# SKA-INAF/caesar-yolo

Measured on AMD Instinct MI355X. Metric: 512x512 tiles/sec over 16k x 16k FITS, higher is better.
Workload: dtype f16

## Files before the change

caesar_yolo_amd/csrc/cy_extra.hip:

```cpp
#include "cy_kernels.h"
#include "cy_conv_dev.h"
#include <cstdlib>

namespace cy {

template <typename T> struct Vec8;
template <> struct Vec8<f16> { typedef f16 type __attribute__((ext_vector_type(8))); };
template <> struct Vec8<float> { typedef float type __attribute__((ext_vector_type(8))); };

template <bool SPLIT, typename T> __device__ __forceinline__ float ld1(const T* p, int lo) {
    if constexpr (SPLIT) return (float)p[0] + (float)p[lo]; else return (float)p[0];
}
template <bool SPLIT, typename T> __device__ __forceinline__ void st1(T* p, int lo, float v) {
    if constexpr (SPLIT) { const T h = (T)v; p[0] = h; p[lo] = (T)(v - (float)h); } else p[0] = (T)v;
}

constexpr int DW_PX = 4;
template <typename T, bool SPLIT = false>
__global__ __launch_bounds__(256) void dwconv3x3_kernel(const DwArgs a) {
    typedef typename Vec8<T>::type v8;
    const int cg = a.C / 8, xb = (a.W + DW_PX - 1) / DW_PX;
    const long total = (long)a.B * a.H * xb * cg;
    const long wg = a.xcd ? xcd_contiguous(blockIdx.x, gridDim.x) : blockIdx.x;
    for (long idx = wg * 256 + threadIdx.x; idx < total; idx += (long)gridDim.x * 256) {
// ... 225 lines not shown
        const int c = (int)(idx % cv) * V;
        const long pix = idx / cv;
        const int w = (int)(pix % a.W), h = (int)((pix / a.W) % a.H), b = (int)(pix / ((long)a.W * a.H));
        const T* base = reinterpret_cast<const T*>(a.src) + a.src_coff + c;
        vec m = *reinterpret_cast<const vec*>(base + (((long)b * a.H + h) * a.W + w) * a.ct);
#pragma unroll
        for (int dh = -2; dh <= 2; ++dh) {
            int hh = h + dh;
            hh = hh < 0 ? 0 : (hh >= a.H ? a.H - 1 : hh);
#pragma unroll
            for (int dw = -2; dw <= 2; ++dw) {
                if (dh == 0 && dw == 0) continue;
                int ww = w + dw;
                ww = ww < 0 ? 0 : (ww >= a.W ? a.W - 1 : ww);
                const vec v = *reinterpret_cast<const vec*>(base + (((long)b * a.H + hh) * a.W + ww) * a.ct);
#pragma unroll
                for (int j = 0; j < V; ++j) m[j] = v[j] > m[j] ? v[j] : m[j];
            }
        }
        *reinterpret_cast<vec*>(reinterpret_cast<T*>(a.dst) + pix * a.ct + a.dst_coff + c) = m;
    }
}

__global__ __launch_bounds__(256) void pool5_x3_kernel(const PoolArgs a) {
    const int cv = a.C / 8;
    const long total = (long)a.B * a.H * a.W * cv;
    for (long idx = (long)xcd_contiguous(blockIdx.x, gridDim.x) * 256 + threadIdx.x; idx < total; idx += (long)gridDim.x * 256) {
        const int c = (int)(idx % cv) * 8;
        const long pix = idx / cv;
        const int w = (int)(pix % a.W), h = (int)((pix / a.W) % a.H), b = (int)(pix / ((long)a.W * a.H));
        float m[8]; f16x8 mh, ml;
        bool first = true;
        for (int dh = -2; dh <= 2; ++dh)
            for (int dw = -2; dw <= 2; ++dw) {
                const int hh = h + dh, ww = w + dw;
                if ((unsigned)hh >= (unsigned)a.H || (unsigned)ww >= (unsigned)a.W) continue;
                const f16* sp = reinterpret_cast<const f16*>(a.src) + (((long)b * a.H + hh) * a.W + ww) * a.ct + a.src_coff + c;
                const f16x8 vh = *reinterpret_cast<const f16x8*>(sp), vl = *reinterpret_cast<const f16x8*>(sp + a.lo);
#pragma unroll
                for (int j = 0; j < 8; ++j) {
                    const float v = (float)vh[j] + (float)vl[j];
                    if (first || v > m[j]) { m[j] = v; mh[j] = vh[j]; ml[j] = vl[j]; }
                }
                first = false;
            }
        f16* dp = reinterpret_cast<f16*>(a.dst) + pix * a.ct + a.dst_coff + c;
// ... 43 lines not shown
```

caesar_yolo_amd/csrc/cy_kernels.h:

```cpp
#pragma once
#include <hip/hip_runtime.h>
#include <stdint.h>
#include <stdlib.h>
#include "cy_measure_jobs.h"
#include "cy_conv_plan.h"

namespace cy {

#ifndef CY_DEV_KNOBS
#define CY_DEV_KNOBS 0
#endif
inline int env_knob(const char* name, int dflt) { const char* e = getenv(name); return e ? atoi(e) : dflt; }
inline int dev_knob(const char* name, int dflt) { return CY_DEV_KNOBS ? env_knob(name, dflt) : dflt; }

template <auto Kernel> void lds_cap(size_t cap) {
    static bool done = false;
    if (done) return;
    (void)hipFuncSetAttribute(reinterpret_cast<const void*>(Kernel), hipFuncAttributeMaxDynamicSharedMemorySize, (int)cap);
    done = true;
}
template <auto Kernel, typename... A> hipError_t launch_lds(dim3 grid, dim3 block, size_t lds, size_t cap, hipStream_t s, A... args) {
    lds_cap<Kernel>(cap);
    hipLaunchKernelGGL(Kernel, grid, block, lds, s, args...);
    return hipGetLastError();
// ... 40 lines not shown
    int xcd;
};
struct AttnArgs {
    const void* qkv; int ct, coff; void* out; int out_ct, out_coff; int B, N, heads, kd, hd; float scale;
    int lo, out_lo;
};
hipError_t launch_dwconv(Precision p, const DwArgs& a, hipStream_t s);
hipError_t launch_attention(Precision p, const AttnArgs& a, hipStream_t s);

hipError_t launch_conv(Precision p, const ConvChoice& choice, const ConvArgs& a, hipStream_t s);
hipError_t launch_head_pair(Precision p, const ConvArgs& a, const ConvArgs& b, hipStream_t s);
void debug_read_stamps(unsigned long long* out8, bool reset);
void debug_read_wg_life(unsigned long long* out, int n);
void debug_read_wg_stamps(unsigned long long* out, int n);
void debug_read_pre_stamps(unsigned long long* out8, bool reset);
void debug_fastdiv(const double* d_a, const double* d_b, double* d_fast, double* d_ref, int n);
void debug_reduce(const double* d_val, const float* d_key, int nrows, int len, unsigned long long* d_out);
hipError_t launch_lds_fill(unsigned pattern, hipStream_t s, int* bytes);
hipError_t launch_stem(Precision p, const StemArgs& a, hipStream_t s);
hipError_t launch_stem_down(const StemDownArgs& a, hipStream_t s);
long stem_down_blocks(const StemDownArgs& a);
void pack_stem_weights2(const float* W, int cout, void* dst);
hipError_t launch_pool5(Precision p, const PoolArgs& a, hipStream_t s);

size_t packed_weight_bytes(Precision p, int cout, int cin, int k, int chunk_bytes = 128);
void pack_weights(Precision p, const float* W, int cout, int cin, int k, void* dst, int chunk_bytes = 128);
void pack_weights_fused2(const float* W2, int cout2, int cin2, void* dst);
int x3_passes(const float* W, int cout, int cin, int k, const float* scale);
size_t packed_weight_bytes_x3(int cout, int cin, int k, int chunk_bytes = 128, int passes = 3);
void pack_weights_x3(const float* W, int cout, int cin, int k, void* dst, float* oscale, int chunk_bytes = 128, int passes = 3, const float* scale = nullptr);
hipError_t launch_x3_split(const float* in, void* out, long npix, int C, hipStream_t s);
hipError_t launch_x3_merge(const void* in, float* out, long npix, int C, hipStream_t s);
void pack_stem_weights(const float* W, int cout, void* dst);
__device__ __forceinline__ int xcd_contiguous(int bid, int nwg) {
    const int q = nwg >> 3, r = nwg & 7, x = bid & 7;
    return (x < r ? x * (q + 1) : r * (q + 1) + (x - r) * q) + (bid >> 3);
}

struct DecodeArgs {
    const float* pred;
    int B, A, nc;
    int lvl_h[3], lvl_w[3];
    float conf;
    float* cand;
    int* cand_anchor;
    int* cand_count;
// ... 237 lines not shown
```

caesar_yolo_amd/csrc/cy_plan.cpp:

```cpp
#include "cy_plan.h"
#include <algorithm>
#include <cmath>
#include <map>

namespace cy {

namespace {
struct Scale { double d, w; int mc; };
bool scale_of(char s, Scale* o) {
    switch (s) {
        case 'n': *o = {0.33, 0.25, 1024}; return true;
        case 's': *o = {0.33, 0.50, 1024}; return true;
        case 'm': *o = {0.67, 0.75, 768}; return true;
        case 'l': *o = {1.00, 1.00, 512}; return true;
        case 'x': *o = {1.00, 1.25, 512}; return true;
    }
    return false;
}
int make_div8(double x) { return (int)std::ceil(x / 8.0) * 8; }

struct Builder {
    Plan p;
    std::map<std::string, int> idx;
    int T(int level, int C) { p.tensors.push_back({level, C}); return (int)p.tensors.size() - 1; }
// ... 337 lines not shown
    if (d2.k != 1 || d2.s != 1 || d2.cin != 256 || d2.cout > 256 || d2.cout % 16) return false;
    if (o.in1 >= 0 || o.up0 || o.res >= 0 || n.res >= 0 || n.c0 != 256) return false;
    if (p.tensors[o.out].level != p.tensors[n.out].level || n.out == o.out) return false;
    return readers_of(p, o.out) == 1;
}

bool box_branch(const Plan& p, size_t i) {
    if (i + 2 >= p.ops.size()) return false;
    const Op& o = p.ops[i]; const Op& n = p.ops[i + 1]; const Op& h = p.ops[i + 2];
    if (o.kind != OPK_CONV || !plain_conv_pair(o, n) || h.kind != OPK_CONV || h.conv < 0) return false;
    const ConvDesc& d0 = p.convs[o.conv]; const ConvDesc& d1 = p.convs[n.conv]; const ConvDesc& d2 = p.convs[h.conv];
    auto c3 = [](const ConvDesc& d) { return d.k == 3 && d.s == 1 && d.act && d.groups == 1 && d.cout == 64; };
    if (!c3(d0) || !c3(d1) || d1.cin != 64 || d0.cin % 64 || o.c0 != d0.cin || n.c0 != 64) return false;
    if (d2.k != 1 || d2.s != 1 || d2.act || d2.groups != 1 || d2.cin != 64 || d2.cout != 64) return false;
    if (o.in1 >= 0 || o.up0 || o.res >= 0 || n.res >= 0 || o.out_coff != 0 || n.out_coff != 0) return false;
    if (h.out >= 0 || h.pred_coff != 0 || h.in0 != n.out || h.in0_coff != 0 || h.c0 != 64 || h.in1 >= 0 || h.up0 || h.res >= 0) return false;
    if (p.tensors[o.out].C != 64 || p.tensors[n.out].C != 64 || o.out == n.out || o.in0 == o.out || o.in0 == n.out) return false;
    const int lev = p.tensors[o.in0].level;
    if (lev != 3 + h.pred_level || p.tensors[o.out].level != lev || p.tensors[n.out].level != lev) return false;
    int writers0 = 0, writers1 = 0;
    for (const Op& q : p.ops) { writers0 += q.out == o.out; writers1 += q.out == n.out; }
    return writers0 == 1 && writers1 == 1 && readers_of(p, o.out) == 1 && readers_of(p, n.out) == 1;
}
}

void mark_fusions(Plan& p) {
    for (size_t i = 0; i < p.ops.size(); ++i) {
        Op& o = p.ops[i];
        o.fuse = FUSE_NONE;
        if (o.box == 0 && box_branch(p, i)) { o.box = 1; p.ops[i + 1].box = 2; p.ops[i + 2].box = 3; }
        if (i + 1 >= p.ops.size()) continue;
        if (bneck_pair(p, i)) o.fuse = FUSE_BNECK_PAIR;
        else if (stem_down_pair(p, i)) o.fuse = FUSE_STEM_DOWN;
        else if (pw_pair(p, i)) o.fuse = FUSE_PW_PAIR;
    }
}

}
```

caesar_yolo_amd/csrc/cy_plan.h:

```cpp
#pragma once
#include <algorithm>
#include <cstddef>
#include <cstdint>
#include <cstring>
#include <string>
#include <vector>

namespace cy {

struct ConvDesc { std::string name; int cin, cout, k, s, act; int groups = 1; };

struct Tensor { int level; int C; };

enum OpKind { OPK_STEM = 0, OPK_CONV = 1, OPK_POOL = 2, OPK_DWCONV = 3, OPK_ATTN = 4 };

enum FuseMark { FUSE_NONE = 0, FUSE_STEM_DOWN, FUSE_PW_PAIR, FUSE_BNECK_PAIR };

struct Op {
    OpKind kind;
    int conv;
    int in0, in0_coff, c0, up0;
    int in1, in1_coff, c1;
    int out, out_coff;
    int res, res_coff;
    int pred_level, pred_coff;
    int p0 = 0, p1 = 0, p2 = 0, p3 = 0;
    FuseMark fuse = FUSE_NONE;
    int box = 0;
};

struct Plan {
    char scale; int nc;
    std::string arch = "yolov8";
    std::vector<ConvDesc> convs;
    std::vector<Tensor> tensors;
    std::vector<Op> ops;
    int feat_level[3];
    bool ok; std::string err;
};

Plan build_plan(char scale, int nc);
int py_round(double x);

struct Reader {
    const unsigned char* p; size_t n, o = 0; bool bad = false;
    uint32_t u32() { if (n - o < 4) { bad = true; return 0; } uint32_t v; memcpy(&v, p + o, 4); o += 4; return v; }
    std::string str(uint32_t len) { if (n - o < len) { bad = true; return ""; } std::string s((const char*)p + o, len); o += std::min<size_t>((len + (size_t)3) / 4 * 4, n - o); return s; }
    const float* f32(size_t cnt) { if ((n - o) / 4 < cnt) { bad = true; return nullptr; } const float* r = (const float*)(p + o); o += 4 * cnt; return r; }
};
struct FileHeader { bool v2 = false, has_flags = false, unsupported = false; uint32_t nconv = 0; std::vector<std::string> names; };
struct ConvRecord { ConvDesc d; const float* W; const float* b; const float* wscale; };
// ... 8 lines not shown
```

caesar_yolo_amd/csrc/cy_runtime.hip:

```cpp
#include "../../include/caesar_yolo_hip.h"
#include "cy_kernels.h"
#include "cy_measure_plan.h"
#include "cy_plan.h"
#include <algorithm>
#include <cmath>
#include <cstdio>
#include <cstdlib>
#include <cstring>
#include <string>
#include <vector>

using namespace cy;

struct DevConv { void* w = nullptr; float* bias = nullptr; size_t wbytes = 0; float* stem_w = nullptr; void* w32 = nullptr; size_t w32bytes = 0;
                 float* oscale = nullptr;
                 void* w2f = nullptr; size_t w2fbytes = 0;
                 int passes = 3;
                 float* dw_w = nullptr;
                 void* bneck = nullptr; };

enum MeasureStep { STEP_SOURCES = 0, STEP_ISLANDS, STEP_DEBLEND, STEP_FIT, STEP_BLEND, STEP_BACKGROUND, STEP_RENDER, STEP_RESIDUAL, STEP_PEAKS, STEP_ATROUS, STEP_APERTURE, STEP_PEAKFIT, STEP_COUNT };

struct DevOwner {
    std::vector<void*> p;
// ... 681 lines not shown
            }
            if (o.out < 0 && o.pred_coff == 0 && c->prec != PREC_F32 && knobs.head_pair && ch.variant == CONV_HEAD_1X1) {
                HeadPend& h = pend[o.pred_level];
                if (h.on) { cur_conv = h.conv; HIPCHK(c, launch_conv(c->prec, h.ch, h.a, s)); prof_done(h.ch.variant, h.flops); cur_conv = o.conv; }
                h.a = a; h.ch = ch; h.flops = flops; h.conv = o.conv; h.on = true;
                return CY_OK;
            }
            if (o.out < 0 && o.pred_coff == 64 && pend[o.pred_level].on) {
                HeadPend& h = pend[o.pred_level];
                h.on = false;
                if (head_pair_ok(c->prec, h.a, h.ch, a, ch, knobs)) {
                    HIPCHK(c, launch_head_pair(c->prec, h.a, a, s));
                    prof_done(CONV_HEAD_1X1, flops + h.flops);
                    return CY_OK;
                }
                cur_conv = h.conv; HIPCHK(c, launch_conv(c->prec, h.ch, h.a, s)); prof_done(h.ch.variant, h.flops); cur_conv = o.conv;
            }
            HIPCHK(c, launch_conv(c->prec, ch, a, s));
            prof_done(ch.variant, flops);
        }
        return CY_OK;
    };
    const size_t n_run = stop > 0 && (size_t)stop < p.ops.size() ? (size_t)stop : p.ops.size();
    size_t i = 0;
    for (; i < n_run; ++i) {
        bool fused = false;
        rc = run_op(p.ops[i], i + 1 < p.ops.size() ? &p.ops[i + 1] : nullptr, &fused);
        if (rc) return rc;
        if (fused) c->fused_last[i++] = 1;
    }
    c->ops_done = (int)(i < p.ops.size() ? i : p.ops.size());
    if (n_run < p.ops.size()) return CY_OK;
    for (HeadPend& h : pend)
        if (h.on) { h.on = false; cur_conv = h.conv; HIPCHK(c, launch_conv(c->prec, h.ch, h.a, s)); prof_done(h.ch.variant, h.flops); }
    if (box_sparse[0] || box_sparse[1] || box_sparse[2]) {
        HIPCHK(c, hipMemsetAsync(bx.L[0].map, 0xFF, (size_t)B * A * sizeof(int), s));
        HIPCHK(c, hipMemsetAsync(bx.L[0].counts, 0, 8 * sizeof(int), s));
        HIPCHK(c, launch_box_mark(bx, s));
        HIPCHK(c, launch_box_sparse(bx, s));
    }
    return CY_OK;
}

int cy_profile_enable(cy_ctx* c, int on) {
    if (!c) return CY_ERR_ARG;
    c->profiling = on != 0;
    c->prof_stride = on > 1 ? on : 1;
    c->fwd_calls = 0;
// ... 317 lines not shown
    if (!ch8(ct) || !ch8(src_coff) || !ch8(dst_coff) || src_coff + C > ct || dst_coff + C > ct)
        return fail(c, CY_ERR_ARG, "channel slice outside its tensor, or an offset / stride not a multiple of 8");
    if (d_src == d_dst && src_coff < dst_coff + C && dst_coff < src_coff + C) return fail(c, CY_ERR_ARG, "overlapping source and destination slices");
    HIPCHK(c, hipSetDevice(c->device));
    hipStream_t st = (hipStream_t)stream;
    const bool x3 = c->prec == PREC_F16X3;
    const int cm = x3 ? 2 : 1;
    const long npix = (long)B * H * W;
    DevOwner sc;
    void *src = const_cast<void*>(d_src), *dst = d_dst;
    hipError_t e = hipSuccess;
    if (x3) e = sc.split(d_dst, npix, ct, &dst, st);
    if (e == hipSuccess && x3) { if (d_src == d_dst) src = dst; else e = sc.split(d_src, npix, ct, &src, st); }
    if (e == hipSuccess) {
        PoolArgs a{};
        a.src = src; a.dst = dst; a.ct = cm * ct; a.src_coff = src_coff; a.dst_coff = dst_coff; a.lo = x3 ? ct : 0;
        a.C = C; a.B = B; a.H = H; a.W = W;
        e = launch_pool5(c->prec, a, st);
    }
    if (e == hipSuccess && x3) e = launch_x3_merge(dst, reinterpret_cast<float*>(d_dst), npix, ct, st);
    return entry_done(c, e, st);
}

int cy_debug_stamps(unsigned long long* out8, int reset) {
    if (!out8) return CY_ERR_ARG;
    if (reset <= -(1 << 20)) { debug_read_wg_life(out8, -reset - (1 << 20)); return CY_OK; }
    if (reset < 0) { debug_read_wg_stamps(out8, -reset); return CY_OK; }
    if (reset >= 2) debug_read_pre_stamps(out8, reset == 3);
    else debug_read_stamps(out8, reset != 0);
    return CY_OK;
}

int cy_debug_fastdiv(const double* d_a, const double* d_b, double* d_fast, double* d_ref, int n) {
    if (!d_a || !d_b || !d_fast || !d_ref || n < 1) return CY_ERR_ARG;
    debug_fastdiv(d_a, d_b, d_fast, d_ref, n);
    return hipGetLastError() == hipSuccess ? CY_OK : CY_ERR_HIP;
}

int cy_debug_reduce(const double* d_val, const float* d_key, int nrows, int len, unsigned long long* d_out) {
    if (!d_out || nrows < 1 || len < 0 || (len > 0 && (!d_val || !d_key))) return CY_ERR_ARG;
    debug_reduce(d_val, d_key, nrows, len, d_out);
    return hipGetLastError() == hipSuccess ? CY_OK : CY_ERR_HIP;
}

int cy_debug_lds_fill(cy_ctx* c, unsigned pattern32, void* stream) {
    if (!c) return CY_ERR_ARG;
// ... 741 lines not shown
```

caesar_yolo_amd/csrc/cy_sparse_box.hip:

```cpp
#include "cy_conv_dev.h"

namespace cy {

namespace {
constexpr int MI = 4, PG = 16 * MI;

__device__ __forceinline__ f16x8 to_mfma_order(const u32x4& v, int src4) {
    u32x4 r;
#pragma unroll
    for (int j = 0; j < 4; ++j) r[j] = (unsigned)__builtin_amdgcn_ds_bpermute(src4, (int)v[j]);
    return __builtin_bit_cast(f16x8, r);
}

template <bool WALK32, int TAPS>
__device__ __forceinline__ void walk(f32x4 (&acc)[4][MI], const unsigned (&xoff)[MI][TAPS], __amdgpu_buffer_rsrc_t rsx, __amdgpu_buffer_rsrc_t rsw,
                                     int nblocks, int lane) {
    static_assert(!WALK32 || TAPS == 9, "the 32-channel walk is the wide 3x3 kernel's");
    constexpr int NS = 2 * TAPS, RING = 3, CPAD = 128;
    const int lr = lane >> 2, lc = lane & 3;
    const int src4 = 4 * (4 * (lane & 15) + (lane >> 4));
    const unsigned wlane = WALK32 ? (unsigned)(lr * 64 + lc * 16) : (unsigned)(lr * 128 + lc * 16);
    u32x4 x[RING][MI], w[RING][4];
    auto load = [&](int slot, int cb, int u) {
        unsigned xs, ws;
// ... 75 lines not shown
        unsigned xoff[MI][9];
#pragma unroll
        for (int mi = 0; mi < MI; ++mi) {
            const int e = g * PG + mi * 16 + lr;
            const int p = e < n ? L.plist[e] : 0;
            const int b = p / HW, r = p - b * HW, y = r / L.W, x = r - y * L.W;
#pragma unroll
            for (int tap = 0; tap < 9; ++tap) {
                const int yy = y + tap / 3 - 1, xx = x + tap % 3 - 1;
                const bool ok = e < n && (unsigned)yy < (unsigned)L.H && (unsigned)xx < (unsigned)L.W;
                xoff[mi][tap] = ok ? (unsigned)((b * HW + yy * L.W + xx) * L.feat_ct + L.feat_coff + lc * 8) * 2u : CY_OOB;
            }
        }
        f32x4 acc[4][MI];
        zero(acc);
        walk<WALK32, 9>(acc, xoff, rsx, rsw, L.cin / 64, lane);
#pragma unroll
        for (int mi = 0; mi < MI; ++mi) {
            const int e = g * PG + mi * 16 + fr;
            if (e < n) act_store<PACKED>(acc, mi, bv, reinterpret_cast<f16*>(L.s1) + (size_t)e * 64 + fq * 16);
        }
    }
}
}

__global__ __launch_bounds__(256) void box_stage1_kernel(const BoxArgs a) {
    const BoxLevel& L = a.L[blockIdx.y];
    if (!L.sparse) return;
    const int lane = threadIdx.x & 63, wid = blockIdx.x * 4 + (threadIdx.x >> 6), nwaves = gridDim.x * 4;
    if (L.walk1 == BOX_WALK_WIDE) stage1<true, true>(L, wid, nwaves, lane);
    else if (L.walk1 == BOX_WALK_PP) stage1<false, false>(L, wid, nwaves, lane);
    else stage1<false, true>(L, wid, nwaves, lane);
}

__global__ __launch_bounds__(256) void box_stage2_kernel(const BoxArgs a) {
    const BoxLevel& L = a.L[blockIdx.y];
    if (!L.sparse) return;
    const int lane = threadIdx.x & 63, fr = lane & 15, fq = lane >> 4, wid = blockIdx.x * 4 + (threadIdx.x >> 6), nwaves = gridDim.x * 4;
    const int n = min(L.counts[1], L.cap), HW = L.H * L.W;
    const auto rsx = __builtin_amdgcn_make_buffer_rsrc(L.s1, 0, (unsigned)L.cap * 128u, 0x00020000);
    const auto rsw = __builtin_amdgcn_make_buffer_rsrc(const_cast<void*>(L.w2), 0, L.w2_bytes, 0x00020000);
    float bv[16];
#pragma unroll
    for (int j = 0; j < 16; ++j) bv[j] = L.b2[fq * 16 + j];
    for (int g = wid; g * PG < n; g += nwaves) {
        unsigned xoff[MI][9];
// ... 40 lines not shown
        }
        f32x4 acc[4][MI];
        zero(acc);
        walk<false, 1>(acc, xoff, rsx, rsw, 1, lane);
#pragma unroll
        for (int mi = 0; mi < MI; ++mi) {
            const int e = g * PG + mi * 16 + fr;
            if (e >= n) continue;
            const int p = L.clist[e], b = p / HW, r = p - b * HW;
            typedef float f32x4u __attribute__((ext_vector_type(4), aligned(4)));
            float* dst = a.pred + ((size_t)b * a.A + L.a_off + r) * (64 + a.nc) + fq * 16;
#pragma unroll
            for (int ni = 0; ni < 4; ++ni)
                *reinterpret_cast<f32x4u*>(dst + 4 * ni) = f32x4u{acc[ni][mi][0] + bv[ni * 4], acc[ni][mi][1] + bv[ni * 4 + 1], acc[ni][mi][2] + bv[ni * 4 + 2],
                                                                  acc[ni][mi][3] + bv[ni * 4 + 3]};
        }
    }
}

hipError_t launch_box_sparse(const BoxArgs& a, hipStream_t s) {
    for (const BoxLevel& L : a.L)
        if (L.sparse && (L.cin % 64 || L.cin < 64 || L.cap < 1 || (size_t)L.cap * 128 >= 0xFFFFFF00ull)) return hipErrorInvalidValue;
    const dim3 grid(BOX_GRID, 3), block(256);
    hipLaunchKernelGGL(box_stage1_kernel, grid, block, 0, s, a);
    hipLaunchKernelGGL(box_stage2_kernel, grid, block, 0, s, a);
    hipLaunchKernelGGL(box_stage3_kernel, grid, block, 0, s, a);
    return hipGetLastError();
}

}
```

caesar_yolo_amd/lib.py:

```python
import ctypes as C
import os

_HERE = os.path.dirname(os.path.abspath(__file__))
LIB_PATH = os.path.join(_HERE, "libcaesar_yolo_hip.so")

CY_MAX_DET = 300
CY_MAX_STAGES = 8
CY_MEAS_FIELDS = 12
MEAS_NAMES = ("npix", "nring", "bkg", "rms", "peak", "x_peak", "y_peak", "sum", "sw", "swx", "swy", "reserved")
CY_ISL_FIELDS = 20
ISL_NAMES = ("status", "nseed", "nislands", "npix", "npix_main", "nborder", "xmin", "xmax", "ymin", "ymax", "S", "Sx", "Sy", "Sxx", "Syy",
             "Sxy", "S_main", "reserved0", "reserved1", "reserved2")
CY_DBL_MAX_COMP, CY_DBL_FIELDS, CY_DBL_COMP_FIELDS = 16, 8, 12
DBL_NAMES = ("status", "nsummits", "npeaks", "ncomp", "npix", "npix_unassigned", "reserved0", "reserved1")
DBL_COMP_NAMES = ("npix", "peak", "x_peak", "y_peak", "S", "Sx", "Sy", "Sxx", "Syy", "Sxy", "main", "nsummits")
CY_FIT_FIELDS = 32
FIT_NAMES = ("status", "niter", "npix", "F", "lambda", "A", "x0", "y0", "a", "b", "c") + tuple(
    "H%d%d" % (i, j) for i in range(6) for j in range(i, 6))
CY_BLEND_FIELDS = 36
CY_BLEND_MAX_MEMBERS = 4
BLEND_NAMES = ("status", "niter", "npix", "F", "lambda", "group", "nmembers", "slot", "A", "x0", "y0", "a", "b", "c", "cov_ok") + tuple(
    "C%d%d" % (i, j) for i in range(6) for j in range(i, 6))
CY_RND_FIELDS, CY_RND_HALF_MAX = 8, 256
RND_NAMES = ("status", "sx0", "sx1", "sy0", "sy1", "ntiles", "reserved0", "reserved1")
# ... 2 lines not shown
             "reserved")
CY_PEAK_FIELDS, CY_PEAK_RADIUS_MAX, CY_PEAK_CAP_MAX = 12, 8, 1 << 20
PEAK_NAMES = ("x", "y", "v", "rms", "snr", "npix", "nabove", "sum", "sw", "swx", "swy", "reserved")
CY_ATROUS_STEP_MAX = 64
CY_APER_RINGS_MAX, CY_APER_RADIUS_MAX, CY_APER_HEAD, CY_APER_RING_FIELDS, CY_APER_JOBS_MAX = 8, 256, 8, 4, 1 << 20
CY_APER_FIELDS = CY_APER_HEAD + CY_APER_RING_FIELDS * CY_APER_RINGS_MAX
APER_NAMES = ("status", "x0", "x1", "y0", "y1", "clipped", "bkg_med", "bkg_mad")
APER_RING_NAMES = ("npix", "sum", "sumsq", "svar")
CY_PFIT_JOB_FIELDS, CY_PFIT_FIELDS, CY_PFIT_RADIUS_MAX, CY_PFIT_NEIGH_MAX, CY_PFIT_JOBS_MAX = 11, 40, 256, 8, 1 << 20
PFIT_JOB_NAMES = ("cx", "cy", "R", "bkg", "sign", "A", "x0", "y0", "a", "b", "c")
PFIT_NAMES = FIT_NAMES + ("wx0", "wx1", "wy0", "wy1", "clipped", "nneigh", "crowded", "nexcluded")
CY_BKG_FIELDS = 8
BKG_NAMES = ("n0", "n", "bkg", "rms", "L", "H", "rounds", "reserved")
OP_BKG, OP_SHIFT, OP_CLIP, OP_ZSCALE, OP_HISTEQ, OP_MINMAX = 1, 2, 3, 4, 5, 6
F16, F32, F16X3 = 0, 1, 2
PRECISIONS = {"fp16": F16, "f16": F16, "half": F16, "fp32": F32, "f32": F32, "float": F32, "fp16x3": F16X3, "f16x3": F16X3, "split": F16X3}

EXPORTS = [
    "cy_create", "cy_destroy", "cy_last_error", "cy_load_weights", "cy_load_weights_mem", "cy_num_classes",
    "cy_weight_passes", "cy_class_name", "cy_plan_num_convs", "cy_plan_conv_desc", "cy_letterbox_geometry", "cy_num_anchors",
    "cy_pred_elems", "cy_profile_enable", "cy_profile_summary", "cy_profile_summary_lane", "cy_profile_layers", "cy_profile_layer_variant", "cy_mosaic_prepare", "cy_letterbox_pack", "cy_preproc", "cy_preproc_planes", "cy_preproc_params", "cy_forward", "cy_debug_read_conv",
    "cy_debug_stop_after", "cy_debug_ops_done", "cy_debug_read_tensor", "cy_debug_sparse_box",
    "cy_decode_nms", "cy_debug_stamps", "cy_debug_fastdiv", "cy_debug_reduce", "cy_debug_lds_fill", "cy_debug_cand_counts", "cy_iou_merge", "cy_detect_tiles", "cy_detect_flush", "cy_detect_fence", "cy_compact_records", "cy_compact_records_ctx", "cy_detect_counters", "cy_conv_bn_silu", "cy_conv_slices", "cy_conv_variant_name", "cy_bottleneck64", "cy_dwconv3x3",
    "cy_attention", "cy_maxpool5", "cy_make_tile_records",
    "cy_merge_edge_sources", "cy_augment_geometry", "cy_enable_augment", "cy_letterbox_pack_f32", "cy_augment_pack",
    "cy_decode_nms_augmented", "cy_detect_tiles_augmented", "cy_measure_sources", "cy_measure_kernel_ms",
    "cy_measure_islands", "cy_islands_kernel_ms", "cy_measure_background", "cy_background_kernel_ms", "cy_expand_background",
    "cy_deblend_islands", "cy_deblend_kernel_ms", "cy_fit_components", "cy_fit_kernel_ms", "cy_fit_blends", "cy_blend_kernel_ms",
    "cy_render_gaussians", "cy_render_kernel_ms", "cy_measure_residuals", "cy_residual_kernel_ms", "cy_find_peaks", "cy_peaks_kernel_ms",
    "cy_atrous_step", "cy_atrous_kernel_ms", "cy_aperture_sums", "cy_aperture_kernel_ms",
    "cy_fit_peaks", "cy_peakfit_kernel_ms",
]


class CyError(RuntimeError):
    pass


class cy_config(C.Structure):
    _fields_ = [("precision", C.c_int), ("max_batch", C.c_int), ("max_h", C.c_int), ("max_w", C.c_int),
                ("max_cand", C.c_int)]


class cy_pre_stage(C.Structure):
    _fields_ = [("op", C.c_int), ("p0", C.c_double), ("p1", C.c_double), ("p2", C.c_double), ("flag", C.c_int)]


# ... 87 lines not shown
        "cy_debug_cand_counts": (C.c_int, [vp, ip, C.c_int]),
        "cy_debug_lds_fill": (C.c_int, [vp, C.c_uint, vp]),
        "cy_debug_stamps": (C.c_int, [C.POINTER(C.c_ulonglong), C.c_int]),
        "cy_debug_fastdiv": (C.c_int, [vp, vp, vp, vp, C.c_int]),
        "cy_debug_reduce": (C.c_int, [vp, vp, C.c_int, C.c_int, vp]),
        "cy_iou_merge": (C.c_int, [vp, vp, vp, C.c_int, C.c_float, C.c_double, C.c_double, vp, vp, vp, vp]),
        "cy_detect_tiles": (C.c_int, [vp, vp, C.c_int, C.c_int, ip, C.c_int, C.c_int, C.c_int, C.c_int,
                                      C.POINTER(cy_preproc_cfg), C.c_float, C.c_float, C.c_double, C.c_double,
                                      vp, vp, vp, vp]),
        "cy_detect_flush": (C.c_int, [vp, vp]),
        "cy_detect_fence": (C.c_int, [vp, vp]),
        "cy_compact_records": (C.c_int, [vp, C.c_longlong, vp, C.c_int, C.c_int, vp, vp, vp]),
        "cy_compact_records_ctx": (C.c_int, [vp, vp, C.c_longlong, vp, C.c_int, C.c_int, vp, vp, vp]),
        "cy_detect_counters": (C.c_int, [vp, C.POINTER(C.c_longlong), C.c_int]),
        "cy_conv_bn_silu": (C.c_int, [vp, vp, C.c_int, C.c_int, C.c_int, C.c_int, fp, fp, C.c_int, C.c_int, C.c_int,
                                      C.c_int, vp, vp, vp]),
        "cy_conv_slices": (C.c_int, [vp, C.POINTER(cy_conv_layout), fp, fp, C.c_char_p, C.c_int, ip, vp]),
        "cy_conv_variant_name": (C.c_char_p, [C.c_int]),
        "cy_bottleneck64": (C.c_int, [vp, vp, C.c_int, C.c_int, C.c_int, fp, fp, fp, fp, C.c_int, vp, vp]),
        "cy_dwconv3x3": (C.c_int, [vp, vp, C.c_int, C.c_int, C.c_int, C.c_int, C.c_int, C.c_int, fp, fp, C.c_int, C.c_int, C.c_int,
                                   C.c_int, vp, C.c_int, C.c_int, vp, C.c_int, C.c_int, vp]),
        "cy_attention": (C.c_int, [vp, vp, C.c_int, C.c_int, C.c_int, C.c_int, C.c_int, C.c_int, C.c_int, vp, C.c_int, C.c_int, vp]),
        "cy_maxpool5": (C.c_int, [vp, vp, C.c_int, C.c_int, C.c_int, C.c_int, C.c_int, C.c_int, vp, C.c_int, vp]),
        "cy_make_tile_records": (C.c_int, [fp, ip, C.c_int, ip, C.c_int, dp]),
        "cy_merge_edge_sources": (C.c_int, [dp, C.c_int, ip, C.c_int, dp]),
        "cy_augment_geometry": (C.c_int, [C.c_int, C.c_int, C.POINTER(cy_augment_geom)]),
        "cy_enable_augment": (C.c_int, [vp]),
        "cy_letterbox_pack_f32": (C.c_int, [vp, vp, C.c_int, C.c_int, C.c_int, C.c_int, vp, vp]),
        "cy_augment_pack": (C.c_int, [vp, vp, C.c_int, C.c_int, C.c_int, vp, vp, vp, vp]),
        "cy_decode_nms_augmented": (C.c_int, [vp, vp, vp, vp, C.c_int, C.c_int, C.c_int, C.c_int, C.c_int, C.c_float, C.c_float,
                                              vp, vp, vp, vp]),
        "cy_detect_tiles_augmented": (C.c_int, [vp, vp, C.c_int, C.c_int, ip, C.c_int, C.c_int, C.c_int, C.c_int,
                                                C.POINTER(cy_preproc_cfg), C.c_float, C.c_float, C.c_double, C.c_double, C.c_int,
                                                vp, vp, vp, vp]),
        "cy_measure_sources": (C.c_int, [vp, vp, C.c_int, C.c_int, dp, C.c_int, C.c_int, dp, vp]),
        "cy_measure_kernel_ms": (C.c_int, [vp, dp]),
        "cy_measure_islands": (C.c_int, [vp, vp, C.c_int, C.c_int, dp, dp, C.c_int, C.c_int, dp, vp, C.POINTER(C.c_longlong), vp]),
        "cy_islands_kernel_ms": (C.c_int, [vp, dp]),
        "cy_deblend_islands": (C.c_int, [vp, vp, C.c_int, C.c_int, dp, dp, C.c_int, C.c_int, C.c_int, dp, dp, vp, C.POINTER(C.c_longlong), vp]),
        "cy_deblend_kernel_ms": (C.c_int, [vp, dp]),
        "cy_fit_components": (C.c_int, [vp, vp, C.c_int, C.c_int, dp, dp, ip, dp, C.c_int, C.c_int, vp, C.POINTER(C.c_longlong), dp, vp]),
        "cy_fit_kernel_ms": (C.c_int, [vp, dp]),
        "cy_fit_blends": (C.c_int, [vp, vp, C.c_int, C.c_int, dp, dp, ip, dp, C.c_int, C.c_int, vp, C.POINTER(C.c_longlong), dp, vp]),
        "cy_blend_kernel_ms": (C.c_int, [vp, dp]),
        "cy_render_gaussians": (C.c_int, [vp, vp, C.c_int, C.c_int, dp, C.c_int, C.c_double, vp, vp, vp, dp, vp]),
        "cy_render_kernel_ms": (C.c_int, [vp, dp]),
# ... 51 lines not shown
```

caesar_yolo_amd/model.py:

```python
import ctypes as C
import logging
import os
import numpy as np
import torch

from . import lib as L
from . import weights as W


_CPU_WARNED = False


def _dev_index(device):
    if isinstance(device, int):
        return device
    s = str(device)
    if s in ("", "cuda", "gpu"):
        return torch.cuda.current_device()
    if s.startswith("cuda:"):
        return int(s.split(":")[1])
    if s.isdigit():
        return int(s)
    if s == "cpu":
        global _CPU_WARNED
# ... 607 lines not shown
    def dwconv3x3(self, x, nch, w, b, out, in_coff=0, out_coff=0, act=True, res=None, res_coff=0, chmap=(0, 0, 0)):
        B, H, Wd, in_ct = x.shape
        w = np.ascontiguousarray(w, np.float32)
        b = np.ascontiguousarray(b, np.float32)
        self._chk(self.lib.cy_dwconv3x3(self.ctx, self._p(x), B, H, Wd, int(nch), in_ct, int(in_coff),
                                        w.ctypes.data_as(C.POINTER(C.c_float)), b.ctypes.data_as(C.POINTER(C.c_float)),
                                        int(bool(act)), int(chmap[0]), int(chmap[1]), int(chmap[2]),
                                        self._p(res) if res is not None else None, res.shape[-1] if res is not None else 0,
                                        int(res_coff), self._p(out), out.shape[-1], int(out_coff), self._stream()))
        return out

    def attention(self, qkv, heads, kd, hd, out, coff=0, out_coff=0):
        B, N, ct = qkv.shape
        self._chk(self.lib.cy_attention(self.ctx, self._p(qkv), B, N, ct, int(coff), int(heads), int(kd), int(hd), self._p(out),
                                        out.shape[-1], int(out_coff), self._stream()))
        return out

    def maxpool5(self, src, nch, dst, src_coff=0, dst_coff=0):
        B, H, Wd, ct = src.shape
        assert tuple(dst.shape) == tuple(src.shape)
        self._chk(self.lib.cy_maxpool5(self.ctx, self._p(src), B, H, Wd, int(nch), ct, int(src_coff), self._p(dst), int(dst_coff),
                                       self._stream()))
        return dst


class _Boxes(object):
    def __init__(self, det):
        self.xyxy, self.conf, self.cls = det[:, :4], det[:, 4], det[:, 5]


class Results(object):
    def __init__(self, det):
        self.boxes = _Boxes(det)


class YOLO(object):

    def __init__(self, weights, precision="fp16x3", max_batch=64, max_imgsz=640, device=None):
        self._wpath = self._resolve(weights)
        self._kw = dict(precision=precision, max_batch=max_batch, max_imgsz=max_imgsz)
        self._det = None
        self._dev = device
        scale, names, _, _ = W.read_cyw_header(self._wpath)
        self.names = names
        self.scale = scale

# ... 86 lines not shown
```

include/caesar_yolo_hip.h:

```cpp
#ifndef CAESAR_YOLO_HIP_H
#define CAESAR_YOLO_HIP_H
#include <stddef.h>
#include <stdint.h>
#ifdef __cplusplus
extern "C" {
#endif

typedef struct cy_ctx cy_ctx;

enum cy_status { CY_OK = 0, CY_ERR_ARG = -1, CY_ERR_HIP = -2, CY_ERR_IO = -3, CY_ERR_STATE = -4, CY_ERR_UNSUPPORTED = -5 };
enum cy_precision { CY_F16 = 0, CY_F32 = 1, CY_F16X3 = 2 };

#define CY_MAX_DET 300
#define CY_DET_STRIDE 6
#define CY_MAX_STAGES 8
#define CY_MAX_CAND 65535

typedef struct cy_config {
    int precision;
    int max_batch;
    int max_h, max_w;
    int max_cand;
} cy_config;

// ... 82 lines not shown

typedef struct cy_conv_layout {
    const void* d_in0; int in0_ct, in0_coff, c0, up0;
    const void* d_in1; int in1_ct, in1_coff, c1;
    const void* d_res; int res_ct, res_coff;
    void* d_out; int out_ct, out_coff;
    int rows, out_bs, out_ro;
    int B, Hi, Wi, Cin, Cout, k, s, act;
} cy_conv_layout;
int cy_conv_slices(cy_ctx* ctx, const cy_conv_layout* layout, const float* h_w, const float* h_b, char* variant,
                   int variant_cap, int* passes, void* stream);
const char* cy_conv_variant_name(int idx);

int cy_bottleneck64(cy_ctx* ctx, const void* d_in, int B, int H, int W, const float* h_w1, const float* h_b1,
                    const float* h_w2, const float* h_b2, int shortcut, void* d_out, void* stream);

int cy_dwconv3x3(cy_ctx* ctx, const void* d_in, int B, int H, int W, int C, int in_ct, int in_coff, const float* h_w,
                 const float* h_b, int act, int blk, int gstride, int goff, const void* d_res, int res_ct, int res_coff,
                 void* d_out, int out_ct, int out_coff, void* stream);
int cy_attention(cy_ctx* ctx, const void* d_qkv, int B, int N, int ct, int coff, int heads, int kd, int hd, void* d_out,
                 int out_ct, int out_coff, void* stream);
int cy_maxpool5(cy_ctx* ctx, const void* d_src, int B, int H, int W, int C, int ct, int src_coff, void* d_dst, int dst_coff,
                void* stream);

typedef struct cy_augment_view {
    double scale; int flip;
    int ch, cw;
    int Hp, Wp;
    int A;
    int lo, hi;
    int off;
} cy_augment_view;
typedef struct cy_augment_geom { cy_augment_view v[3]; int total; } cy_augment_geom;
int cy_augment_geometry(int H, int W, cy_augment_geom* out);
int cy_enable_augment(cy_ctx* ctx);
int cy_letterbox_pack_f32(cy_ctx* ctx, const double* d_planes, int B, int h0, int w0, int imgsz, float* d_out, void* stream);
int cy_augment_pack(cy_ctx* ctx, const float* d_src, int B, int H, int W, void* d_view0, void* d_view1, void* d_view2, void* stream);
int cy_decode_nms_augmented(cy_ctx* ctx, const float* d_pred0, const float* d_pred1, const float* d_pred2, int B, int H, int W,
                            int h0, int w0, float conf, float iou, float* d_det, int* d_det_anchor, int* d_count, void* stream);
int cy_detect_tiles_augmented(cy_ctx* ctx, const float* d_mosaic, int MH, int MW, const int* h_tiles, int B, int th, int tw,
                              int imgsz, const cy_preproc_cfg* cfg, float conf, float iou, double thr_soft, double thr_hard,
                              int augment, float* d_out, int* d_out_count, int* d_status, void* stream);

#define CY_MEAS_FIELDS 12
int cy_measure_sources(cy_ctx* ctx, const float* d_img, int MH, int MW, const double* h_boxes, int n, int ring,
                       double* h_out , void* stream);
// ... 98 lines not shown
```

Measured before the change: 9166.

## Fuse SPPF triple maxpool into one LDS kernel and stage box weights via LDS

Adds a kernel that runs the three chained 5x5 maxpools of the SPPF block in one launch. Each workgroup holds one image's channel group in LDS as order-preserving integer keys, with an exact float fallback for NaN and signed-zero cases. This removes two launches and the global round trips between the pools. Separately, the sparse box stage-1 kernel now defaults to a variant that streams weights through an LDS ring via DMA, with a 3-slot pipeline. Both paths are enabled by default through env knobs and add complexity around LDS size limits and NaN handling.

```diff
diff --git a/caesar_yolo_amd/csrc/cy_extra.hip b/caesar_yolo_amd/csrc/cy_extra.hip
--- a/caesar_yolo_amd/csrc/cy_extra.hip
+++ b/caesar_yolo_amd/csrc/cy_extra.hip
@@ -271,6 +271,90 @@
     }
 }
 
+template <typename T> struct PoolKey;
+template <> struct PoolKey<f16> { typedef short I; static constexpr int INF = 0x7C00; };
+template <> struct PoolKey<float> { typedef int I; static constexpr int INF = 0x7F800000; };
+
+template <typename T>
+__global__ __launch_bounds__(256) void sppf_pool5_kernel(const PoolArgs a) {
+    constexpr int V = 16 / sizeof(T);
+    typedef T vec __attribute__((ext_vector_type(V)));
+    typedef typename PoolKey<T>::I I;
+    typedef I ivec __attribute__((ext_vector_type(V)));
+    constexpr I SIGN_SHIFT = 8 * sizeof(T) - 1, INF = (I)PoolKey<T>::INF, MAG = (I)(PoolKey<T>::INF | (PoolKey<T>::INF - 1));
+    auto key = [](ivec x) -> ivec { return x ^ ((x >> SIGN_SHIFT) & MAG); };
+    extern __shared__ __attribute__((aligned(16))) unsigned char sppf_planes[];
+    const int cv = a.C / V, ng = (cv + SPPF_GV - 1) / SPPF_GV;
+    const int wg = xcd_contiguous(blockIdx.x, gridDim.x);
+    const int b = wg / ng, g = wg - b * ng;
+    const int nv = cv - g * SPPF_GV < SPPF_GV ? cv - g * SPPF_GV : SPPF_GV;
+    const int hw = a.H * a.W, n = hw * nv;
+    ivec* cur = reinterpret_cast<ivec*>(sppf_planes);
+    ivec* nxt = cur + n;
+    T* img = reinterpret_cast<T*>(a.dst) + (long)b * hw * a.ct + g * (SPPF_GV * V);
+    for (int i = threadIdx.x; i < n; i += 256) {
+        const int pix = i / nv, v = i - pix * nv;
+        cur[i] = key(*reinterpret_cast<const ivec*>(img + (long)pix * a.ct + a.src_coff + v * V));
+    }
+    __syncthreads();
+#pragma unroll
+    for (int j = 0; j < 3; ++j) {
+        T* out = img + a.dst_coff + j * a.C;
+        for (int i = threadIdx.x; i < n; i += 256) {
+            const int pix = i / nv, v = i - pix * nv;
+            const int h = pix / a.W, w = pix - h * a.W;
+            int row[5], col[5];
+#pragma unroll
+            for (int d = 0; d < 5; ++d) {
+                const int hh = h + d - 2, ww = w + d - 2;
+                row[d] = (hh < 0 ? 0 : (hh >= a.H ? a.H - 1 : hh)) * a.W * nv + v;
+                col[d] = (ww < 0 ? 0 : (ww >= a.W ? a.W - 1 : ww)) * nv;
+            }
+            const ivec c = cur[i];
+            ivec m = c;
+#pragma unroll
+            for (int dh = 0; dh < 5; ++dh)
+#pragma unroll
+                for (int dw = 0; dw < 5; ++dw)
+                    if (dh != 2 || dw != 2) m = __builtin_elementwise_max(m, cur[row[dh] + col[dw]]);
+            const ivec odd = (((m + (I)1) & (I)~1) == (I)0) | (m > INF) | (c < (I)~INF);
+            bool exact = false;
+#pragma unroll
+            for (int e = 0; e < V; ++e) exact |= odd[e] != 0;
+            if (exact) {
+                vec f = __builtin_bit_cast(vec, key(c));
+#pragma unroll 1
+                for (int dh = -2; dh <= 2; ++dh)
+#pragma unroll 1
+                    for (int dw = -2; dw <= 2; ++dw) {
+                        if (dh == 0 && dw == 0) continue;
+                        int hh = h + dh, ww = w + dw;
+                        hh = hh < 0 ? 0 : (hh >= a.H ? a.H - 1 : hh);
+                        ww = ww < 0 ? 0 : (ww >= a.W ? a.W - 1 : ww);
+                        const vec x = __builtin_bit_cast(vec, key(cur[(hh * a.W + ww) * nv + v]));
+#pragma unroll
+                        for (int e = 0; e < V; ++e) f[e] = x[e] > f[e] ? x[e] : f[e];
+                    }
+                m = key(__builtin_bit_cast(ivec, f));
+            }
+            *reinterpret_cast<ivec*>(out + (long)pix * a.ct + v * V) = key(m);
+            if (j < 2) nxt[i] = m;
+        }
+        __syncthreads();
+        ivec* t = cur; cur = nxt; nxt = t;
+    }
+}
+
+hipError_t launch_sppf_pool5(Precision p, const PoolArgs& a, hipStream_t s) {
+    if (!sppf_pool5_ok(p, a) || a.src != a.dst) return hipErrorInvalidValue;
+    const int V = p == PREC_F16 ? 8 : 4;
+    const long grid = (long)a.B * ((a.C / V + SPPF_GV - 1) / SPPF_GV);
+    if (grid < 1 || grid > 0x7fffffffL) return hipErrorInvalidValue;
+    if (p == PREC_F16) hipLaunchKernelGGL(sppf_pool5_kernel<f16>, dim3((unsigned)grid), dim3(256), sppf_pool5_lds(a), s, a);
+    else hipLaunchKernelGGL(sppf_pool5_kernel<float>, dim3((unsigned)grid), dim3(256), sppf_pool5_lds(a), s, a);
+    return hipGetLastError();
+}
+
 __global__ __launch_bounds__(256) void pool5_x3_kernel(const PoolArgs a) {
     const int cv = a.C / 8;
     const long total = (long)a.B * a.H * a.W * cv;
diff --git a/caesar_yolo_amd/csrc/cy_kernels.h b/caesar_yolo_amd/csrc/cy_kernels.h
--- a/caesar_yolo_amd/csrc/cy_kernels.h
+++ b/caesar_yolo_amd/csrc/cy_kernels.h
@@ -86,6 +86,13 @@
 long stem_down_blocks(const StemDownArgs& a);
 void pack_stem_weights2(const float* W, int cout, void* dst);
 hipError_t launch_pool5(Precision p, const PoolArgs& a, hipStream_t s);
+constexpr int SPPF_GV = 4;
+constexpr size_t SPPF_LDS_MAX = 64 * 1024;
+inline size_t sppf_pool5_lds(const PoolArgs& a) { return (size_t)a.H * a.W * (2 * SPPF_GV * 16); }
+inline bool sppf_pool5_ok(Precision p, const PoolArgs& a) {
+    return p != PREC_F16X3 && a.C > 0 && a.C % (p == PREC_F16 ? 8 : 4) == 0 && sppf_pool5_lds(a) <= SPPF_LDS_MAX;
+}
+hipError_t launch_sppf_pool5(Precision p, const PoolArgs& a, hipStream_t s);
 
 size_t packed_weight_bytes(Precision p, int cout, int cin, int k, int chunk_bytes = 128);
 void pack_weights(Precision p, const float* W, int cout, int cin, int k, void* dst, int chunk_bytes = 128);
diff --git a/caesar_yolo_amd/csrc/cy_plan.cpp b/caesar_yolo_amd/csrc/cy_plan.cpp
--- a/caesar_yolo_amd/csrc/cy_plan.cpp
+++ b/caesar_yolo_amd/csrc/cy_plan.cpp
@@ -383,12 +383,27 @@
     for (const Op& q : p.ops) { writers0 += q.out == o.out; writers1 += q.out == n.out; }
     return writers0 == 1 && writers1 == 1 && readers_of(p, o.out) == 1 && readers_of(p, n.out) == 1;
 }
+
+bool sppf_chain(const Plan& p, size_t i) {
+    if (i + 2 >= p.ops.size()) return false;
+    const Op& a = p.ops[i]; const Op& b = p.ops[i + 1]; const Op& c = p.ops[i + 2];
+    if (a.kind != OPK_POOL || b.kind != OPK_POOL || c.kind != OPK_POOL) return false;
+    const int t = a.in0, C = a.c0;
+    if (t < 0 || a.out != t || b.in0 != t || b.out != t || c.in0 != t || c.out != t || b.c0 != C || c.c0 != C) return false;
+    if (C < 8 || C % 8 || p.tensors[t].C % 8 || a.in0_coff < 0 || a.in0_coff % 8 || a.out_coff < 0 || a.out_coff % 8) return false;
+    if (b.in0_coff != a.out_coff || (long)b.out_coff != (long)a.out_coff + C) return false;
+    if (c.in0_coff != b.out_coff || (long)c.out_coff != (long)b.out_coff + C) return false;
+    if ((long)a.out_coff + 3L * C > p.tensors[t].C || (long)a.in0_coff + C > p.tensors[t].C) return false;
+    return (long)a.in0_coff + C <= a.out_coff || (long)a.out_coff + 3L * C <= a.in0_coff;
+}
 }
 
 void mark_fusions(Plan& p) {
+    for (Op& o : p.ops) o.sppf = 0;
     for (size_t i = 0; i < p.ops.size(); ++i) {
         Op& o = p.ops[i];
         o.fuse = FUSE_NONE;
+        if (o.sppf == 0 && sppf_chain(p, i)) { o.sppf = 1; p.ops[i + 1].sppf = 2; p.ops[i + 2].sppf = 3; }
         if (o.box == 0 && box_branch(p, i)) { o.box = 1; p.ops[i + 1].box = 2; p.ops[i + 2].box = 3; }
         if (i + 1 >= p.ops.size()) continue;
         if (bneck_pair(p, i)) o.fuse = FUSE_BNECK_PAIR;
diff --git a/caesar_yolo_amd/csrc/cy_plan.h b/caesar_yolo_amd/csrc/cy_plan.h
--- a/caesar_yolo_amd/csrc/cy_plan.h
+++ b/caesar_yolo_amd/csrc/cy_plan.h
@@ -27,6 +27,7 @@
     int p0 = 0, p1 = 0, p2 = 0, p3 = 0;
     FuseMark fuse = FUSE_NONE;
     int box = 0;
+    int sppf = 0;
 };
 
 struct Plan {
diff --git a/caesar_yolo_amd/csrc/cy_runtime.hip b/caesar_yolo_amd/csrc/cy_runtime.hip
--- a/caesar_yolo_amd/csrc/cy_runtime.hip
+++ b/caesar_yolo_amd/csrc/cy_runtime.hip
@@ -727,8 +727,28 @@
         return CY_OK;
     };
     const size_t n_run = stop > 0 && (size_t)stop < p.ops.size() ? (size_t)stop : p.ops.size();
+    const int sppf_env = env_knob("CY_SPPF_FUSE", 1);
+    auto run_sppf = [&](size_t at, bool* done) -> int {
+        const Op& o = p.ops[at];
+        const Tensor& t = p.tensors[o.in0];
+        PoolArgs a{};
+        a.dst = tptr(o.in0); a.src = a.dst; a.ct = t.C; a.src_coff = o.in0_coff; a.dst_coff = o.out_coff;
+        a.C = o.c0; a.B = B; a.H = H >> t.level; a.W = W >> t.level;
+        if (!sppf_pool5_ok(c->prec, a)) return CY_OK;
+        cur_conv = -1;
+        HIPCHK(c, launch_sppf_pool5(c->prec, a, s));
+        prof_done(CONV_NUM_VARIANTS + 1, 0.0);
+        *done = true;
+        return CY_OK;
+    };
     size_t i = 0;
     for (; i < n_run; ++i) {
+        if (sppf_env && p.ops[i].sppf == 1 && i + 3 <= n_run) {
+            bool done = false;
+            rc = run_sppf(i, &done);
+            if (rc) return rc;
+            if (done) { i += 2; continue; }
+        }
         bool fused = false;
         rc = run_op(p.ops[i], i + 1 < p.ops.size() ? &p.ops[i + 1] : nullptr, &fused);
         if (rc) return rc;
@@ -1092,6 +1112,33 @@
     return entry_done(c, e, st);
 }
 
+int cy_sppf_pool5(cy_ctx* c, void* d_buf, int B, int H, int W, int C, int ct, int src_coff, int dst_coff, int* launches, void* stream) {
+    if (!c || !d_buf) return fail(c, CY_ERR_ARG, "null argument");
+    if (c->prec == PREC_F16X3) return fail(c, CY_ERR_UNSUPPORTED, "the fp16x3 context runs the SPPF chain pool by pool (cy_maxpool5)");
+    if (B < 1 || H < 1 || W < 1 || C < 8 || C % 8) return fail(c, CY_ERR_ARG, "unsupported pool geometry");
+    if (!ch8(ct) || !ch8(src_coff) || !ch8(dst_coff) || src_coff + C > ct || (long)dst_coff + 3L * C > ct)
+        return fail(c, CY_ERR_ARG, "channel slice outside its tensor, or an offset / stride not a multiple of 8");
+    if (src_coff < dst_coff + 3 * C && dst_coff < src_coff + C) return fail(c, CY_ERR_ARG, "overlapping source and destination slices");
+    HIPCHK(c, hipSetDevice(c->device));
+    hipStream_t st = (hipStream_t)stream;
+    PoolArgs a{};
+    a.src = d_buf; a.dst = d_buf; a.ct = ct; a.src_coff = src_coff; a.dst_coff = dst_coff; a.C = C; a.B = B; a.H = H; a.W = W;
+    hipError_t e = hipSuccess;
+    int n = 0;
+    if (env_knob("CY_SPPF_FUSE", 1) && sppf_pool5_ok(c->prec, a)) {
+        e = launch_sppf_pool5(c->prec, a, st);
+        n = 1;
+    } else {
+        for (int j = 0; j < 3 && e == hipSuccess; ++j, ++n) {
+            PoolArgs q = a;
+            q.src_coff = j == 0 ? src_coff : dst_coff + (j - 1) * C; q.dst_coff = dst_coff + j * C;
+            e = launch_pool5(c->prec, q, st);
+        }
+    }
+    if (launches) *launches = n;
+    return entry_done(c, e, st);
+}
+
 int cy_debug_stamps(unsigned long long* out8, int reset) {
     if (!out8) return CY_ERR_ARG;
     if (reset <= -(1 << 20)) { debug_read_wg_life(out8, -reset - (1 << 20)); return CY_OK; }
diff --git a/caesar_yolo_amd/csrc/cy_sparse_box.hip b/caesar_yolo_amd/csrc/cy_sparse_box.hip
--- a/caesar_yolo_amd/csrc/cy_sparse_box.hip
+++ b/caesar_yolo_amd/csrc/cy_sparse_box.hip
@@ -121,6 +121,109 @@
         }
     }
 }
+
+template <bool WALK32>
+__device__ __forceinline__ void walk_lds(f32x4 (&acc)[4][MI], const unsigned (&xoff)[MI][9], __amdgpu_buffer_rsrc_t rsx, __amdgpu_buffer_rsrc_t rsw,
+                                         int nblocks, int lane, int wave, char* ring) {
+    constexpr int TAPS = 9, NS = 2 * TAPS, RING = 3, CPAD = 128, STEP = 4096, ROWB = WALK32 ? 64 : 128;
+    static_assert(NS % RING == 0, "ring slots are compile-time per step");
+    const int fr = lane & 15, fq = lane >> 4, lr = lane >> 2, lc = lane & 3;
+    const int src4 = 4 * (4 * (lane & 15) + (lane >> 4));
+    const unsigned wreq = (unsigned)((wave * 16 + lr) * ROWB + ((lc ^ (((lr >> 2) & 1) << 1)) << 4));
+    const unsigned wrd = (unsigned)(fr * 64 + ((fq ^ (((fr >> 2) & 1) << 1)) << 4));
+    u32x4 x[RING][MI];
+    auto request = [&](int slot, int cb, int u) {
+        unsigned xs, ws;
+        int tap;
+        if constexpr (WALK32) {
+            const int slab = 2 * cb + u / 9;
+            tap = u % 9;
+            xs = (unsigned)slab * 64u;
+            ws = (unsigned)((slab * 9 + tap) * CPAD) * 64u;
+        } else {
+            const int kk = u & 1;
+            tap = u >> 1;
+            xs = (unsigned)cb * 128u + (unsigned)kk * 64u;
+            ws = (unsigned)((cb * TAPS + tap) * CPAD) * 128u + (unsigned)kk * 64u;
+        }
+        dma_piece(rsw, (lds_ptr_t*)(ring + slot * STEP + wave * 1024), wreq, ws);
+#pragma unroll
+        for (int mi = 0; mi < MI; ++mi) x[slot][mi] = load_b128(rsx, xoff[mi][tap], xs);
+    };
+    request(0, 0, 0);
+    request(1, 0, 1);
+#pragma unroll 1
+    for (int cb = 0; cb < nblocks; ++cb) {
+        const bool more = cb + 1 < nblocks;
+#pragma unroll
+        for (int u = 0; u < NS; ++u) {
+            if (u == NS - 1 && !more) { CY_WAIT_VM(MI); } else { CY_WAIT_VM(2 * MI + 1); }
+            __builtin_amdgcn_sched_barrier(0);
+            __builtin_amdgcn_s_barrier();
+            __builtin_amdgcn_sched_barrier(0);
+            if (u + 2 < NS) request((u + 2) % RING, cb, u + 2);
+            else if (more) request((u + 2) % RING, cb + 1, u + 2 - NS);
+            f16x8 wf[4], xf[MI];
+#pragma unroll
+            for (int ni = 0; ni < 4; ++ni) wf[ni] = *reinterpret_cast<const f16x8*>(ring + (u % RING) * STEP + ni * 1024 + wrd);
+#pragma unroll
+            for (int mi = 0; mi < MI; ++mi) xf[mi] = to_mfma_order(x[u % RING][mi], src4);
+#pragma unroll
+            for (int ni = 0; ni < 4; ++ni)
+#pragma unroll
+                for (int mi = 0; mi < MI; ++mi) acc[ni][mi] = __builtin_amdgcn_mfma_f32_16x16x32_f16(wf[ni], xf[mi], acc[ni][mi], 0, 0, 0);
+            asm volatile("s_waitcnt lgkmcnt(0)" ::: "memory");
+        }
+    }
+}
+
+template <bool WALK32, bool PACKED>
+__device__ __forceinline__ void stage1_lds(const BoxLevel& L, int lane, int wave, char* ring) {
+    const int fr = lane & 15, fq = lane >> 4, lr = lane >> 2, lc = lane & 3;
+    const int n = __builtin_amdgcn_readfirstlane(min(L.counts[0], L.cap));
+    const int HW = L.H * L.W;
+    const auto rsx = __builtin_amdgcn_make_buffer_rsrc(const_cast<void*>(L.feat), 0, L.feat_bytes, 0x00020000);
+    const auto rsw = __builtin_amdgcn_make_buffer_rsrc(const_cast<void*>(L.w1), 0, L.w1_bytes, 0x00020000);
+    float bv[16];
+#pragma unroll
+    for (int j = 0; j < 16; ++j) bv[j] = L.b1[fq * 16 + j];
+    const int nwaves = (int)gridDim.x * 4;
+    for (int gb = (int)blockIdx.x * 4; gb * PG < n; gb += nwaves) {
+        const int g = gb + wave;
+        unsigned xoff[MI][9];
+#pragma unroll
+        for (int mi = 0; mi < MI; ++mi) {
+            const int e = g * PG + mi * 16 + lr;
+            const int p = e < n ? L.plist[e] : 0;
+            const int b = p / HW, r = p - b * HW, y = r / L.W, x = r - y * L.W;
+#pragma unroll
+            for (int tap = 0; tap < 9; ++tap) {
+                const int yy = y + tap / 3 - 1, xx = x + tap % 3 - 1;
+                const bool ok = e < n && (unsigned)yy < (unsigned)L.H && (unsigned)xx < (unsigned)L.W;
+                xoff[mi][tap] = ok ? (unsigned)((b * HW + yy * L.W + xx) * L.feat_ct + L.feat_coff + lc * 8) * 2u : CY_OOB;
+            }
+        }
+        f32x4 acc[4][MI];
+        zero(acc);
+        CY_WAIT_VM(0);
+        walk_lds<WALK32>(acc, xoff, rsx, rsw, L.cin / 64, lane, wave, ring);
+#pragma unroll
+        for (int mi = 0; mi < MI; ++mi) {
+            const int e = g * PG + mi * 16 + fr;
+            if (e < n) act_store<PACKED>(acc, mi, bv, reinterpret_cast<f16*>(L.s1) + (size_t)e * 64 + fq * 16);
+        }
+    }
+}
+}
+
+__global__ __launch_bounds__(256) void box_stage1_lds_kernel(const BoxArgs a) {
+    __shared__ __attribute__((aligned(16))) char ring[3 * 4096];
+    const BoxLevel& L = a.L[blockIdx.y];
+    if (!L.sparse) return;
+    const int lane = threadIdx.x & 63, wave = __builtin_amdgcn_readfirstlane(threadIdx.x >> 6);
+    if (L.walk1 == BOX_WALK_WIDE) stage1_lds<true, true>(L, lane, wave, ring);
+    else if (L.walk1 == BOX_WALK_PP) stage1_lds<false, false>(L, lane, wave, ring);
+    else stage1_lds<false, true>(L, lane, wave, ring);
 }
 
 __global__ __launch_bounds__(256) void box_stage1_kernel(const BoxArgs a) {
@@ -207,7 +310,8 @@
     for (const BoxLevel& L : a.L)
         if (L.sparse && (L.cin % 64 || L.cin < 64 || L.cap < 1 || (size_t)L.cap * 128 >= 0xFFFFFF00ull)) return hipErrorInvalidValue;
     const dim3 grid(BOX_GRID, 3), block(256);
-    hipLaunchKernelGGL(box_stage1_kernel, grid, block, 0, s, a);
+    if (env_knob("CY_BOX_LDS_W", 1)) hipLaunchKernelGGL(box_stage1_lds_kernel, grid, block, 0, s, a);
+    else hipLaunchKernelGGL(box_stage1_kernel, grid, block, 0, s, a);
     hipLaunchKernelGGL(box_stage2_kernel, grid, block, 0, s, a);
     hipLaunchKernelGGL(box_stage3_kernel, grid, block, 0, s, a);
     return hipGetLastError();
diff --git a/caesar_yolo_amd/lib.py b/caesar_yolo_amd/lib.py
--- a/caesar_yolo_amd/lib.py
+++ b/caesar_yolo_amd/lib.py
@@ -48,7 +48,7 @@
     "cy_pred_elems", "cy_profile_enable", "cy_profile_summary", "cy_profile_summary_lane", "cy_profile_layers", "cy_profile_layer_variant", "cy_mosaic_prepare", "cy_letterbox_pack", "cy_preproc", "cy_preproc_planes", "cy_preproc_params", "cy_forward", "cy_debug_read_conv",
     "cy_debug_stop_after", "cy_debug_ops_done", "cy_debug_read_tensor", "cy_debug_sparse_box",
     "cy_decode_nms", "cy_debug_stamps", "cy_debug_fastdiv", "cy_debug_reduce", "cy_debug_lds_fill", "cy_debug_cand_counts", "cy_iou_merge", "cy_detect_tiles", "cy_detect_flush", "cy_detect_fence", "cy_compact_records", "cy_compact_records_ctx", "cy_detect_counters", "cy_conv_bn_silu", "cy_conv_slices", "cy_conv_variant_name", "cy_bottleneck64", "cy_dwconv3x3",
-    "cy_attention", "cy_maxpool5", "cy_make_tile_records",
+    "cy_attention", "cy_maxpool5", "cy_sppf_pool5", "cy_make_tile_records",
     "cy_merge_edge_sources", "cy_augment_geometry", "cy_enable_augment", "cy_letterbox_pack_f32", "cy_augment_pack",
     "cy_decode_nms_augmented", "cy_detect_tiles_augmented", "cy_measure_sources", "cy_measure_kernel_ms",
     "cy_measure_islands", "cy_islands_kernel_ms", "cy_measure_background", "cy_background_kernel_ms", "cy_expand_background",
@@ -182,6 +182,7 @@
                                    C.c_int, vp, C.c_int, C.c_int, vp, C.c_int, C.c_int, vp]),
         "cy_attention": (C.c_int, [vp, vp, C.c_int, C.c_int, C.c_int, C.c_int, C.c_int, C.c_int, C.c_int, vp, C.c_int, C.c_int, vp]),
         "cy_maxpool5": (C.c_int, [vp, vp, C.c_int, C.c_int, C.c_int, C.c_int, C.c_int, C.c_int, vp, C.c_int, vp]),
+        "cy_sppf_pool5": (C.c_int, [vp, vp, C.c_int, C.c_int, C.c_int, C.c_int, C.c_int, C.c_int, C.c_int, C.POINTER(C.c_int), vp]),
         "cy_make_tile_records": (C.c_int, [fp, ip, C.c_int, ip, C.c_int, dp]),
         "cy_merge_edge_sources": (C.c_int, [dp, C.c_int, ip, C.c_int, dp]),
         "cy_augment_geometry": (C.c_int, [C.c_int, C.c_int, C.POINTER(cy_augment_geom)]),
diff --git a/caesar_yolo_amd/model.py b/caesar_yolo_amd/model.py
--- a/caesar_yolo_amd/model.py
+++ b/caesar_yolo_amd/model.py
@@ -653,6 +653,13 @@
         self._chk(self.lib.cy_maxpool5(self.ctx, self._p(src), B, H, Wd, int(nch), ct, int(src_coff), self._p(dst), int(dst_coff),
                                        self._stream()))
         return dst
+
+    def sppf_pool5(self, buf, nch, src_coff, dst_coff):
+        B, H, Wd, ct = buf.shape
+        n = C.c_int(0)
+        self._chk(self.lib.cy_sppf_pool5(self.ctx, self._p(buf), B, H, Wd, int(nch), ct, int(src_coff), int(dst_coff), C.byref(n),
+                                         self._stream()))
+        return n.value
 
 
 class _Boxes(object):
diff --git a/include/caesar_yolo_hip.h b/include/caesar_yolo_hip.h
--- a/include/caesar_yolo_hip.h
+++ b/include/caesar_yolo_hip.h
@@ -128,6 +128,8 @@
                  int out_ct, int out_coff, void* stream);
 int cy_maxpool5(cy_ctx* ctx, const void* d_src, int B, int H, int W, int C, int ct, int src_coff, void* d_dst, int dst_coff,
                 void* stream);
+int cy_sppf_pool5(cy_ctx* ctx, void* d_buf, int B, int H, int W, int C, int ct, int src_coff, int dst_coff, int* launches,
+                  void* stream);
 
 typedef struct cy_augment_view {
     double scale; int flip;
```

Measured after the change: 9212, median of 6. No clear change (+0.5%).
